# MCG-NJU/LinK

Measured on AMD Instinct MI355X. Metric: voxels/s through one LinK (3x7)^3 block, 100k active voxels C=64, higher is better.
Workload: dtype f32

## Files before the change

include/link_amd.h:

```cpp
#ifndef LINK_AMD_H_
#define LINK_AMD_H_

#include <stddef.h>
#include <stdint.h>

#ifdef __cplusplus
extern "C" {
#endif

#define LINK_OK 0
#define LINK_ERR_ARG (-1)
#define LINK_ERR_LAUNCH (-2)
#define LINK_ERR_WORKSPACE (-3)
#define LINK_BATCH_TIMEOUT (-4)

int link_abi_version(void);
int32_t link_abi_struct_size(int32_t which);
const char *link_last_error(void);


int link_hash(const int32_t *coords, int64_t n, int64_t *out, void *stream);

int link_kernel_hash(const int32_t *coords, int64_t n, const int32_t *offsets, int64_t k,
                     int64_t *out, void *stream);
// ... 427 lines not shown
  int32_t subm;
  int32_t *nbr;
  int32_t *pair_arena;
  int64_t pair_arena_words;
  float *contrib;
  int64_t contrib_rows;
  const float *w;
  const void *ws;
  const int32_t *w_big;
  const float *nl_w, *nl_b;
  float nl_eps;
  int32_t flags;
  void *out;
  int32_t bbox[8];
  int32_t stats[4];
  int32_t verdict;
  int32_t reserved;
} link_block_args_t;
int link_elk_block_forward(link_block_ctx_t *ctx, link_block_args_t *args , void *stream);

typedef struct link_dc_batch link_dc_batch_t;
int link_dc_batch_create(link_dc_batch_t **out);
int link_dc_batch_destroy(link_dc_batch_t *ctx);
int link_elk_core_dense_forward_batch(link_dc_batch_t *ctx, const link_dc_buffers_t *frames ,
                                      const int64_t *n , int32_t nframes, const link_dc_grid_t *g ,
                                      const link_elk_desc_t *desc , void *stream);
int link_dc_batch_submit(link_dc_batch_t *ctx, const link_dc_buffers_t *frames , const int64_t *n ,
                         int32_t nframes, const link_dc_grid_t *g , const link_elk_desc_t *desc , void *stream,
                         int64_t *ticket );
int link_dc_batch_join(link_dc_batch_t *ctx, int64_t ticket, void *stream);
int link_dc_batch_status(link_dc_batch_t *ctx, int32_t *out );
int link_dc_batch_set_timing(link_dc_batch_t *ctx, int32_t on);
int link_dc_batch_kernel_times(link_dc_batch_t *ctx, int64_t ticket, float *ms );
int link_dc_batch_set_debug(link_dc_batch_t *ctx, uint64_t *k1_rows, uint64_t *k2_rows);
int link_streams_share_queue(void *stream_a, void *stream_b, double *delay_us );
int link_dc_batch_probe_streams(link_dc_batch_t *ctx, hipStream_t stream, double *delays_us );

#define LINK_NMS_ROTATE 0
#define LINK_NMS_NORMAL 1
#define LINK_NMS_CIRCLE 2
int link_boxes_overlap_bev(const float *boxes_a, int64_t na, const float *boxes_b, int64_t nb, float *out , void *stream);
int link_boxes_iou_bev(const float *boxes_a, int64_t na, const float *boxes_b, int64_t nb, float *out , void *stream);
size_t link_nms_workspace_bytes(int64_t n);
int link_nms_mask(const float *boxes, int64_t cap, const int32_t *n_dev, int32_t pred, float thr, uint64_t *mask, void *stream);
int link_nms_reduce(const uint64_t *mask, int64_t cap, const int32_t *n_dev, int32_t post_max, int64_t *keep ,
                    int32_t *count , void *stream);
int link_nms_bev(const float *boxes, int64_t cap, const int32_t *n_dev, int32_t pred, float thr, int32_t post_max, void *workspace,
                 size_t workspace_bytes, int64_t *keep , int32_t *count , void *stream);
typedef struct {
  float out_size_factor, voxel_size[2], pc_range[2], score_threshold, post_center_range[6];
} link_center_geom_t;
int link_center_decode(const float *hm, const float *reg, const float *height, const float *dim, const float *rot, const float *vel,
                       int32_t batch, int32_t num_cls, int32_t h, int32_t w, const link_center_geom_t *geom , float *boxes,
                       int32_t *labels, float *scores, int32_t *counts, void *stream);

#define LINK_VOXELIZE_HARD 0
#define LINK_VOXELIZE_DYNAMIC 1
typedef struct {
  float lo[3], hi[3], vs[3];
  int32_t grid[3];
  int32_t max_points, max_voxels, ndim, mode;
} link_voxelize_geom_t;
size_t link_voxelize_workspace_bytes(const link_voxelize_geom_t *geom , int64_t n_points_capacity, int32_t batch);
int link_voxelize(const link_voxelize_geom_t *geom , const float *points, const int32_t *point_offsets ,
                  int32_t batch, int64_t n_points_capacity, void *workspace, size_t workspace_bytes, float *voxels ,
                  float *mean, int32_t *coors , int32_t *num_points, int64_t voxel_capacity,
// ... 144 lines not shown
```

link_amd/_lib.py:

```python
from __future__ import annotations

import ctypes
import os
from ctypes import POINTER, Structure, c_char_p, c_double, c_float, c_int, c_int32, c_int64, c_size_t, c_void_p

_HERE = os.path.dirname(os.path.abspath(__file__))
SO_PATH = os.path.join(_HERE, "lib", "liblink_amd.so")

LINK_OK, LINK_ERR_ARG, LINK_ERR_LAUNCH, LINK_ERR_WORKSPACE, LINK_BATCH_TIMEOUT = 0, -1, -2, -3, -4
HDR_M, HDR_STATUS, HDR_NVALID, HDR_STATUS_ACC, HDR_WORDS = 0, 1, 2, 3, 8
OP_COS, OP_SIN, OP_COSX = 0, 1, 2
ELK_LANE_CHANNEL, ELK_NO_PAIR, ELK_FUSED_GATHER, ELK_NO_DENSE_GRID, ELK_TILES = 1, 2, 4, 8, 16
ELK_LEAN_CS, ELK_LEAN_NO_CS, ELK_LEAN_PM, ELK_LEAN_NO_PM = 32, 64, 128, 256
IO_F32, IO_F16, IO_BF16 = 0, 1, 2
ABI_VERSION = 13
DEBUG = os.environ.get("LINK_AMD_DEBUG", "0") not in ("", "0")


class LinkGrid(Structure):
    _fields_ = [("s", c_int32), ("lo", c_int32 * 4), ("dim", c_int32 * 4)]

    @property
    def cells(self) -> int:
        v = 1
# ... 255 lines not shown
    "link_bn_apply_backward_io": (c_int, [c_void_p, c_void_p, c_int32] + [c_void_p] * 4 + [c_int64, c_int32, c_void_p, c_void_p]),
    "link_elk_mid_partial_rows": (c_int32, []),
    "link_dc_grid_from": (c_int64, [POINTER(LinkGrid), c_int32, POINTER(LinkDcGrid)]),
    "link_dc_premix_insert": (c_int, [c_void_p] * 5 + [c_int64, c_int32, c_float, POINTER(LinkDcGrid), c_int32] +
                              [c_void_p] * 7),
    "link_dc_modsum": (c_int, [c_void_p] * 6 + [POINTER(LinkElkDesc), POINTER(LinkDcGrid), c_int32, c_void_p,
                               c_void_p, c_void_p]),
    "link_dc_gather": (c_int, [c_void_p, c_void_p, POINTER(LinkElkDesc), POINTER(LinkDcGrid), c_void_p, c_void_p]),
    "link_elk_core_dense_forward": (c_int, [POINTER(LinkDcBuffers), POINTER(LinkDcGrid), POINTER(LinkElkDesc),
                                            c_int64, c_int32, c_void_p]),
    "link_elk_core_lean_forward": (c_int, [POINTER(LinkLeanBuffers), POINTER(LinkGrid), POINTER(LinkElkDesc), c_int64, c_int64,
                                           c_int32, c_void_p]),
    "link_dc_index_probe": (c_int, [POINTER(LinkDcBuffers), POINTER(LinkDcGrid), c_int64, c_void_p, c_void_p]),
    "link_dc_index_ids": (c_int, [c_void_p, c_int64, POINTER(LinkDcGrid)] + [c_void_p] * 5),
    "link_dc_index": (c_int, [c_void_p, c_int64, POINTER(LinkDcGrid)] + [c_void_p] * 5),
    "link_dc_premix_modsum": (c_int, [POINTER(LinkDcBuffers), POINTER(LinkDcGrid), POINTER(LinkElkDesc), c_int64,
                                      c_int32, c_void_p]),
    "link_dc_gather_demod": (c_int, [POINTER(LinkDcBuffers), POINTER(LinkDcGrid), POINTER(LinkElkDesc), c_int64, c_void_p]),
    "link_dc_demod": (c_int, [c_void_p] * 8 + [POINTER(LinkElkDesc), POINTER(LinkDcGrid), c_int64, c_void_p, c_int32,
                              c_void_p]),
    "link_block_ctx_create": (c_int, [POINTER(c_void_p)]),
    "link_block_ctx_destroy": (c_int, [c_void_p]),
    "link_pair_plan_arena": (c_int64, [c_int64, c_int32, c_int32, POINTER(c_int64)]),
    "link_dc_neighbor_map": (c_int, [c_void_p, c_int64, POINTER(LinkDcGrid), c_void_p, c_void_p, c_int32, c_void_p, c_void_p]),
    "link_elk_block_forward": (c_int, [c_void_p, POINTER(LinkBlockArgs), c_void_p]),
    "link_dc_batch_create": (c_int, [POINTER(c_void_p)]),
    "link_dc_batch_destroy": (c_int, [c_void_p]),
    "link_elk_core_dense_forward_batch": (c_int, [c_void_p, POINTER(LinkDcBuffers), POINTER(c_int64), c_int32, POINTER(LinkDcGrid),
                                                  POINTER(LinkElkDesc), c_void_p]),
    "link_dc_batch_submit": (c_int, [c_void_p, POINTER(LinkDcBuffers), POINTER(c_int64), c_int32, POINTER(LinkDcGrid),
                                     POINTER(LinkElkDesc), c_void_p, POINTER(c_int64)]),
    "link_dc_batch_join": (c_int, [c_void_p, c_int64, c_void_p]),
    "link_dc_batch_set_timing": (c_int, [c_void_p, c_int32]),
    "link_dc_batch_kernel_times": (c_int, [c_void_p, c_int64, POINTER(c_float)]),
    "link_dc_batch_status": (c_int, [c_void_p, POINTER(c_int32)]),
    "link_dc_batch_set_debug": (c_int, [c_void_p, c_void_p, c_void_p]),
    "link_dc_batch_probe_streams": (c_int, [c_void_p, c_void_p, POINTER(ctypes.c_double)]),
    "link_streams_share_queue": (c_int, [c_void_p, c_void_p, POINTER(ctypes.c_double)]),
    "link_elk_mid_backward": (c_int, [c_void_p] * 9 + [POINTER(LinkGrid), c_void_p, c_void_p, c_void_p,
                                      POINTER(LinkElkDesc), c_int64, c_int64] + [c_void_p] * 5),
    "link_boxes_overlap_bev": (c_int, [c_void_p, c_int64, c_void_p, c_int64, c_void_p, c_void_p]),
    "link_boxes_iou_bev": (c_int, [c_void_p, c_int64, c_void_p, c_int64, c_void_p, c_void_p]),
    "link_nms_workspace_bytes": (c_size_t, [c_int64]),
    "link_nms_mask": (c_int, [c_void_p, c_int64, c_void_p, c_int32, c_float, c_void_p, c_void_p]),
    "link_nms_reduce": (c_int, [c_void_p, c_int64, c_void_p, c_int32, c_void_p, c_void_p, c_void_p]),
    "link_nms_bev": (c_int, [c_void_p, c_int64, c_void_p, c_int32, c_float, c_int32, c_void_p, c_size_t, c_void_p, c_void_p, c_void_p]),
    "link_center_decode": (c_int, [c_void_p] * 6 + [c_int32] * 4 + [POINTER(LinkCenterGeom)] + [c_void_p] * 5),
    "link_voxelize_workspace_bytes": (c_size_t, [POINTER(LinkVoxelizeGeom), c_int64, c_int32]),
    "link_voxelize": (c_int, [POINTER(LinkVoxelizeGeom), c_void_p, c_void_p, c_int32, c_int64, c_void_p, c_size_t] + [c_void_p] * 4 +
                      [c_int64, c_void_p, c_void_p]),
    "link_segloss_workspace_bytes": (c_size_t, [c_int64, c_int32]),
    "link_segloss_forward": (c_int, [c_void_p, c_int32, c_int32, c_void_p, c_int64, c_int32, c_int64, c_int64, c_int32, c_int32, c_void_p,
                                     c_size_t, c_void_p, c_void_p, c_void_p]),
    "link_segloss_backward": (c_int, [c_void_p, c_void_p, c_int64, c_int32, c_int32, c_void_p, c_void_p]),
    "link_center_assign": (c_int, [POINTER(LinkCenterAssignGeom), c_void_p, c_void_p, c_int32, c_int32] + [POINTER(c_void_p)] * 5 + [c_void_p]),
    "link_center_loss_workspace_bytes": (c_size_t, [c_int32] * 5),
    "link_center_loss_forward": (c_int, [c_void_p] * 6 + [POINTER(c_int64), c_int32, c_int32] + [c_void_p] * 5 + [c_int32] * 5 + [POINTER(c_float), c_float, c_void_p,
                                         c_size_t, c_void_p, c_void_p, c_void_p, c_void_p]),
    "link_center_loss_backward": (c_int, [c_void_p] * 5 + [c_int32] * 6 + [c_void_p] * 6 + [POINTER(c_int64), c_void_p]),
    "link_seg_quantize_workspace_bytes": (c_size_t, [c_int64, c_int32]),
    "link_seg_quantize": (c_int, [c_void_p, c_int32, c_int32, c_float, c_void_p, c_int32, c_int64, c_void_p, c_size_t, c_void_p, c_void_p,
                                  c_int64] + [c_void_p] * 5),
    "link_seg_vote_eval": (c_int, [c_void_p, c_int32, c_int32, c_int64, c_int32, c_void_p, c_int32, c_int64, c_void_p, c_int64] +
                           [c_void_p] * 4),
    "link_tta_views": (c_int, [c_void_p, c_void_p, c_int32, c_int64, c_int32, c_float, c_float, c_void_p, c_void_p, c_void_p]),
    "link_center_decode_flip4": (c_int, [c_void_p] * 6 + [c_int32] * 4 + [POINTER(LinkCenterGeom)] + [c_void_p] * 5),
# ... 84 lines not shown
```

link_amd/csrc/dense_batch.hip:

```cpp
#define DC_IO 0
#define DC_IO_NS dcb_f32
#include "dense_batch_impl.h"

namespace dcb_f16 { int batch_set_launch(const link::dc_bt_host_t &, const link_dc_buffers_t *, const int64_t *, int, const link_dc_grid_t &, const link_elk_desc_t &); }
namespace dcb_bf16 { int batch_set_launch(const link::dc_bt_host_t &, const link_dc_buffers_t *, const int64_t *, int, const link_dc_grid_t &, const link_elk_desc_t &); }

using namespace link;
using namespace dcb_f32;

static constexpr int BT_RING = 4;
__global__ void k_dc_batch_spin(unsigned long long *stamp, int ticks) {
  const unsigned long long t0 = __builtin_amdgcn_s_memrealtime();
  if (threadIdx.x == 0) *stamp = t0;
  while (__builtin_amdgcn_s_memrealtime() - t0 < (unsigned long long)ticks) __builtin_amdgcn_s_sleep(16);
}
static bool bt_queue_delay_us(hipStream_t x, hipStream_t y, unsigned long long *scratch , hipEvent_t ev, double *us) {
  unsigned long long h[2] = {0, 0};
  *us = 0.0;
  if (hipStreamSynchronize(x) != hipSuccess || hipStreamSynchronize(y) != hipSuccess) return false;
  hipLaunchKernelGGL(k_dc_batch_spin, dim3(1), dim3(64), 0, x, scratch, 15000);
  if (hipEventRecord(ev, x) != hipSuccess) return false;
  hipLaunchKernelGGL(k_dc_batch_spin, dim3(1), dim3(64), 0, y, scratch + 1, 0);
  if (hipStreamSynchronize(x) != hipSuccess || hipStreamSynchronize(y) != hipSuccess ||
      hipMemcpy(h, scratch, sizeof h, hipMemcpyDeviceToHost) != hipSuccess)
    return false;
  *us = ((double)h[1] - (double)h[0]) / 100.0;
  return true;
}
static bool bt_share_queue(hipStream_t x, hipStream_t y, unsigned long long *scratch, hipEvent_t ev) {
  double d = 0.0;
  return !bt_queue_delay_us(x, y, scratch, ev, &d) || d > 75.0;
}
struct link_dc_batch {
  int device, cus;
  hipStream_t sa, sb, sc;
  std::vector<hipStream_t> pool;
  int ia, ib;
  std::vector<std::pair<hipStream_t, unsigned>> callers;
  unsigned long long *probe_scratch;
  hipEvent_t probe_ev;
  bool timing;
  hipEvent_t tb[BT_RING][3], te[BT_RING][3];
  bool timed[BT_RING];
  int32_t *sync;
  hipEvent_t ev_in[BT_RING], ev_ms[BT_RING], ev_a[BT_RING], ev_c[BT_RING], ev_out[BT_RING];
  std::vector<const void *> bufs[BT_RING];
  bool used[BT_RING];
  long long calls;
  unsigned long long *dbg1, *dbg2;
};

extern "C" int link_dc_batch_create(link_dc_batch_t **out) {
  if (!out) return LINK_ERR_ARG;
  link_dc_batch *c = new link_dc_batch();
  hipDeviceProp_t pr;
  if (hipGetDevice(&c->device) != hipSuccess || hipGetDeviceProperties(&pr, c->device) != hipSuccess) { delete c; return LINK_ERR_LAUNCH; }
  c->cus = pr.multiProcessorCount;
  int pr_lo = 0, pr_hi = 0;
  (void)hipDeviceGetStreamPriorityRange(&pr_lo, &pr_hi);
  bool ok = hipStreamCreateWithPriority(&c->sc, hipStreamNonBlocking, pr_hi) == hipSuccess &&
            hipMalloc(reinterpret_cast<void **>(&c->probe_scratch), 16) == hipSuccess &&
            hipEventCreateWithFlags(&c->probe_ev, hipEventDisableTiming) == hipSuccess;
  std::vector<hipStream_t> rejected;
  const bool dbg_place = getenv("LINK_DC_BATCH_DEBUG") != nullptr;
  for (int cand = 0; ok && cand < 12 && c->pool.size() < 4; cand++) {
    hipStream_t s_ = nullptr;
    if (hipStreamCreateWithFlags(&s_, hipStreamNonBlocking) != hipSuccess) { ok = false; break; }
    bool bad = bt_share_queue(c->sc, s_, c->probe_scratch, c->probe_ev);
    for (size_t i = 0; i < c->pool.size() && !bad; i++) bad = bt_share_queue(c->pool[i], s_, c->probe_scratch, c->probe_ev);
    (bad ? rejected : c->pool).push_back(s_);
  }
  while (ok && c->pool.size() < 2 && !rejected.empty()) { c->pool.push_back(rejected.back()); rejected.pop_back(); }
  for (hipStream_t s_ : rejected) (void)hipStreamDestroy(s_);
  ok = ok && c->pool.size() >= 2;
  if (ok) { c->ia = 0; c->ib = 1; c->sa = c->pool[0]; c->sb = c->pool[1]; }
  if (dbg_place)
    fprintf(stderr, "link_dc_batch_create: %zu streams on hardware queues of their own, %zu candidates rejected\n",
            c->pool.size(), rejected.size());
  ok = ok && hipMalloc(reinterpret_cast<void **>(&c->sync), sizeof(int32_t) * BT_RING * BT_SYNC_WORDS) == hipSuccess &&
            hipMemset(c->sync, 0, sizeof(int32_t) * BT_RING * BT_SYNC_WORDS) == hipSuccess;
  for (int i = 0; i < BT_RING && ok; i++) {
#ifndef DC_BT_EVENT_FLAGS
#define DC_BT_EVENT_FLAGS (hipEventDisableTiming | hipEventDisableSystemFence)
#endif
    ok = hipEventCreateWithFlags(&c->ev_in[i], DC_BT_EVENT_FLAGS) == hipSuccess && hipEventCreateWithFlags(&c->ev_ms[i], DC_BT_EVENT_FLAGS) == hipSuccess &&
         hipEventCreateWithFlags(&c->ev_a[i], DC_BT_EVENT_FLAGS) == hipSuccess && hipEventCreateWithFlags(&c->ev_c[i], DC_BT_EVENT_FLAGS) == hipSuccess &&
         hipEventCreateWithFlags(&c->ev_out[i], DC_BT_EVENT_FLAGS) == hipSuccess;
    c->used[i] = false;
  }
  c->calls = 0;
  c->dbg1 = c->dbg2 = nullptr;
  if (!ok) { (void)hipGetLastError(); delete c; return LINK_ERR_LAUNCH; }
  *out = c;
  return LINK_OK;
}

extern "C" int link_dc_batch_destroy(link_dc_batch_t *c) {
  if (!c) return LINK_OK;
  (void)hipStreamSynchronize(c->sa); (void)hipStreamSynchronize(c->sb); (void)hipStreamSynchronize(c->sc);
  for (int i = 0; i < BT_RING; i++) {
    (void)hipEventDestroy(c->ev_in[i]); (void)hipEventDestroy(c->ev_ms[i]); (void)hipEventDestroy(c->ev_a[i]); (void)hipEventDestroy(c->ev_c[i]);
    (void)hipEventDestroy(c->ev_out[i]);
  }
  for (int i = 0; i < BT_RING; i++)
    for (int k = 0; k < 3; k++) { if (c->tb[i][k]) (void)hipEventDestroy(c->tb[i][k]); if (c->te[i][k]) (void)hipEventDestroy(c->te[i][k]); }
  (void)hipFree(c->sync);
  (void)hipFree(c->probe_scratch);
  (void)hipEventDestroy(c->probe_ev);
  for (hipStream_t s_ : c->pool) (void)hipStreamDestroy(s_);
  (void)hipStreamDestroy(c->sc);
  delete c;
  return LINK_OK;
}

extern "C" int link_dc_batch_set_debug(link_dc_batch_t *c, uint64_t *k1_rows, uint64_t *k2_rows) {
  if (!c) return LINK_ERR_ARG;
  c->dbg1 = reinterpret_cast<unsigned long long *>(k1_rows);
  c->dbg2 = reinterpret_cast<unsigned long long *>(k2_rows);
  return DC_BT_PROF ? LINK_OK : 1;
}

extern "C" int link_streams_share_queue(void *a, void *b, double *delay_us) {
  if (!delay_us) return LINK_ERR_ARG;
  unsigned long long *st = nullptr;
  hipEvent_t ev;
  if (hipMalloc(reinterpret_cast<void **>(&st), 16) != hipSuccess) return LINK_ERR_LAUNCH;
  if (hipEventCreateWithFlags(&ev, hipEventDisableTiming) != hipSuccess) { (void)hipFree(st); return LINK_ERR_LAUNCH; }
  const bool ok = bt_queue_delay_us(S(a), S(b), st, ev, delay_us);
  (void)hipEventDestroy(ev);
  (void)hipFree(st);
  if (!ok) { (void)hipGetLastError(); return LINK_ERR_LAUNCH; }
  return LINK_OK;
}

extern "C" int link_dc_batch_probe_streams(link_dc_batch_t *c, hipStream_t caller, double *delays_us ) {
  if (!c || !delays_us) return LINK_ERR_ARG;
  unsigned long long *st = nullptr;
  hipEvent_t ev;
  if (hipMalloc(reinterpret_cast<void **>(&st), 16) != hipSuccess) return LINK_ERR_LAUNCH;
  if (hipEventCreateWithFlags(&ev, hipEventDisableTiming) != hipSuccess) { (void)hipFree(st); return LINK_ERR_LAUNCH; }
  hipStream_t xs[12] = {c->sa, c->sa, c->sb, caller, caller, caller, c->sb, c->sc, c->sc, c->sa, c->sb, c->sc},
              ys[12] = {c->sb, c->sc, c->sc, c->sa, c->sb, c->sc, c->sa, c->sa, c->sb, caller, caller, caller};
  bool ok = true;
  for (int i = 0; i < 12; i++) ok = bt_queue_delay_us(xs[i], ys[i], st, ev, &delays_us[i]) && ok;
// ... 93 lines not shown
    for (int i = 0; i < nb; i++) keys.push_back(frames[base + i].S);
    bool fail = hipEventRecord(c->ev_in[q], st) != hipSuccess;
    fail = fail || hipStreamWaitEvent(c->sa, c->ev_in[q], 0) != hipSuccess || hipStreamWaitEvent(c->sb, c->ev_in[q], 0) != hipSuccess ||
           hipStreamWaitEvent(c->sc, c->ev_in[q], 0) != hipSuccess;
    for (int r = 0; r < BT_RING && !fail; r++) {
      if (!c->used[r]) continue;
      bool dep = r == q;
      for (size_t i = 0; i < keys.size() && !dep; i++)
        for (size_t k = 0; k < c->bufs[r].size() && !dep; k++) dep = keys[i] == c->bufs[r][k];
      if (dep)
        fail = hipStreamWaitEvent(c->sa, c->ev_out[r], 0) != hipSuccess || hipStreamWaitEvent(c->sc, c->ev_out[r], 0) != hipSuccess ||
               hipStreamWaitEvent(c->sa, c->ev_a[r], 0) != hipSuccess || hipStreamWaitEvent(c->sc, c->ev_a[r], 0) != hipSuccess;
    }
    int32_t *sync = c->sync + (size_t)q * BT_SYNC_WORDS;
#ifndef DC_BT_CLEAR_ON_INSERT
#define DC_BT_CLEAR_ON_INSERT 1
#endif
    hipStream_t s_clear = DC_BT_CLEAR_ON_INSERT ? c->sc : c->sa, s_o1 = DC_BT_CLEAR_ON_INSERT ? c->sa : c->sc;
    if (!fail) hipLaunchKernelGGL(k_dc_batch_clear, dim3(1), dim3(256), 0, s_clear, sync, (int)BT_SYNC_WORDS);
    fail = fail || hipEventRecord(c->ev_ms[q], s_clear) != hipSuccess ||
           hipStreamWaitEvent(c->sb, c->ev_ms[q], 0) != hipSuccess || hipStreamWaitEvent(s_o1, c->ev_ms[q], 0) != hipSuccess;
    if (fail) { (void)hipGetLastError(); return LINK_ERR_LAUNCH; }
    int rc;
    hipStream_t role3[3] = {c->sc, c->sa, c->sb};
    c->timed[q] = false;
    if (c->timing) {
      bool okt = true;
      for (int i = 0; i < 3 && okt; i++) {
        if (!c->tb[q][i]) okt = hipEventCreate(&c->tb[q][i]) == hipSuccess && hipEventCreate(&c->te[q][i]) == hipSuccess;
        okt = okt && hipEventRecord(c->tb[q][i], role3[i]) == hipSuccess;
      }
      c->timed[q] = okt;
    }
    const dc_bt_host_t hset{c->sa, c->sb, c->sc, c->cus, sync, c->dbg1, c->dbg2};
    if (b0.io_dtype == LINK_IO_F16) rc = dcb_f16::batch_set_launch(hset, frames + base, n + base, nb, *g, *d);
    else if (b0.io_dtype == LINK_IO_BF16) rc = dcb_bf16::batch_set_launch(hset, frames + base, n + base, nb, *g, *d);
    else rc = dcb_f32::batch_set_launch(hset, frames + base, n + base, nb, *g, *d);
    if (c->timed[q])
      for (int i = 0; i < 3; i++) c->timed[q] = hipEventRecord(c->te[q][i], role3[i]) == hipSuccess && c->timed[q];
    fail = hipEventRecord(c->ev_a[q], c->sa) != hipSuccess || hipEventRecord(c->ev_c[q], c->sc) != hipSuccess || hipEventRecord(c->ev_out[q], c->sb) != hipSuccess;
    c->bufs[q] = keys;
    c->used[q] = true;
    if (ticket) *ticket = c->calls;
    c->calls++;
    if (rc != LINK_OK || fail) {
      (void)hipStreamWaitEvent(st, c->ev_a[q], 0); (void)hipStreamWaitEvent(st, c->ev_c[q], 0); (void)hipStreamWaitEvent(st, c->ev_out[q], 0);
      if (rc != LINK_OK) return rc;
      (void)hipGetLastError();
      return LINK_ERR_LAUNCH;
    }
  }
  return LINK_OK;
}

extern "C" int link_dc_batch_join(link_dc_batch_t *c, int64_t ticket, void *stream) {
  if (!c || ticket < 0 || ticket >= c->calls) return LINK_ERR_ARG;
  const int q = (int)(ticket % BT_RING);
  hipStream_t st = S(stream);
  if (hipStreamWaitEvent(st, c->ev_a[q], 0) != hipSuccess || hipStreamWaitEvent(st, c->ev_c[q], 0) != hipSuccess ||
      hipStreamWaitEvent(st, c->ev_out[q], 0) != hipSuccess) {
    (void)hipGetLastError();
    return LINK_ERR_LAUNCH;
  }
  return LINK_OK;
}

extern "C" int link_elk_core_dense_forward_batch(link_dc_batch_t *c, const link_dc_buffers_t *frames, const int64_t *n, int32_t nframes,
// ... 7 lines not shown
```

link_amd/csrc/dense_batch_common.h:

```cpp
#pragma once
#include <hip/hip_runtime.h>
#include <stdint.h>

#include "link_amd.h"

#ifndef DC_BT_MAX
#define DC_BT_MAX 48
#endif
#ifndef DC_BT_TIMEOUT_TICKS
#define DC_BT_TIMEOUT_TICKS 200000000ull
#endif
#ifndef DC_BT_PROF
#define DC_BT_PROF 0
#endif
#ifndef DC_BT_INS_LEAD
#define DC_BT_INS_LEAD 1000
#endif
#ifndef DC_BT_INS_WAVES
#define DC_BT_INS_WAVES 4
#endif
#ifndef DC_BT_RELEASE_FENCE
#define DC_BT_RELEASE_FENCE 0
#endif
#ifndef DC_BT_K1_WRITEBACK
#define DC_BT_K1_WRITEBACK 0
#endif

namespace link {
__host__ __device__ constexpr int bt_err() { return 0; }
__host__ __device__ constexpr int bt_cursor(int xcd) { return 16 * (1 + xcd); }
__host__ __device__ constexpr int bt_k1cur(int xcd) { return 16 * (9 + xcd); }
__host__ __device__ constexpr int bt_inscur() { return 16 * 17; }
__host__ __device__ constexpr int bt_ins(int f) { return 16 * (18 + 2 * f); }
__host__ __device__ constexpr int bt_k1(int f) { return 16 * (19 + 2 * f); }
constexpr int BT_SYNC_WORDS = 16 * (18 + 2 * DC_BT_MAX);
struct dc_bt_host_t {
  hipStream_t sa, sb, sc;
  int cus;
  int32_t *sync;
  unsigned long long *dbg1, *dbg2;
};
}
```

link_amd/csrc/dense_batch_impl.h:

```cpp
#include <stdlib.h>

#include <type_traits>
#include <vector>

#include "dense_batch_common.h"
#include "dense_gather.h"
#include "dense_io.h"

namespace DC_IO_NS {
using namespace link;

#include "dense_k1_impl.h"
#include "dense_k2_cfg.h"
#include "dense_gather_quad_impl.h"

static_assert(DC_ST_AUX == 16, "the S rows must leave the L2 (sc1) for the in-launch hand-off K1 -> K2");

struct dc_bt_frame_t {
  const void *feats; const int4 *coords; int4 *slots; uint32_t *cnt; int32_t *cell_n; int32_t *vcell; float *S; int32_t *hdr;
  void *out; int64_t n;
};
struct dc_bt_frames_t { dc_bt_frame_t f[DC_BT_MAX]; };
struct dc_bt_par_t {
  const float *w_pre, *pre_ln_w, *pre_ln_b, *w_pos, *ln_w, *ln_b;
  int cg; float eps;
  unsigned long long *dbg1, *dbg2;
};
__device__ __forceinline__ void bt_row(unsigned long long *dbg, unsigned long long r, unsigned long long a, unsigned long long b,
                                       unsigned long long c, unsigned long long d, unsigned long long e, unsigned long long f) {
  if (!DC_BT_PROF || !dbg) return;
  if (r + 1 >= dbg[1]) return;
  unsigned long long *o = dbg + 8 * (r + 1);
  o[0] = a; o[1] = b; o[2] = c; o[3] = d; o[4] = e; o[5] = f; o[6] = 1;
}


template <typename P>
__device__ __forceinline__ bool bt_wait_ge(P sync, int word, int target, const int nap = 8) {
  int ok = 1;
  if ((threadIdx.x & 63) == 0) {
    const unsigned long long t0 = __builtin_amdgcn_s_memrealtime();
    int spins = 0;
    while (__hip_atomic_load(&sync[word], __ATOMIC_RELAXED, __HIP_MEMORY_SCOPE_AGENT) < target) {
      if (nap > 8) __builtin_amdgcn_s_sleep(64); else __builtin_amdgcn_s_sleep(8);
      if ((++spins & 15) == 0) {
        if (__hip_atomic_load(&sync[bt_err()], __ATOMIC_RELAXED, __HIP_MEMORY_SCOPE_AGENT) != 0) { ok = 0; break; }
        if (__builtin_amdgcn_s_memrealtime() - t0 > DC_BT_TIMEOUT_TICKS) {
          __hip_atomic_store(&sync[bt_err()], 1 + word, __ATOMIC_RELAXED, __HIP_MEMORY_SCOPE_AGENT);
          ok = 0;
          break;
        }
      }
    }
  }
  return __builtin_amdgcn_readfirstlane(ok) != 0;
}

struct dc_bt_ins_args_t { dc_bt_frames_t fr; link_dc_grid_t g; int nframes, wpf; int32_t *sync; };
__global__ void __launch_bounds__(64) k_dc_batch_insert(dc_bt_ins_args_t args_by_value) {
  (void)args_by_value;
#if defined(__HIP_DEVICE_COMPILE__)
  typedef const __attribute__((address_space(4))) dc_bt_ins_args_t *args_ptr_t;
  for (;;) {
    args_ptr_t a = (args_ptr_t)__builtin_amdgcn_kernarg_segment_ptr();
    asm volatile("" : "+s"(a));
    int t = 0;
    if (threadIdx.x == 0) t = __hip_atomic_fetch_add(&a->sync[bt_inscur()], 1, __ATOMIC_RELAXED, __HIP_MEMORY_SCOPE_AGENT);
    t = __builtin_amdgcn_readfirstlane(t);
    const int wpf = a->wpf;
    if (t >= a->nframes * wpf) break;
    const int f = t / wpf, j = t - f * wpf;
    if (f >= DC_BT_INS_LEAD && !bt_wait_ge(a->sync, bt_k1(f - DC_BT_INS_LEAD), 1, 64)) break;
    const link_dc_grid_t g = a->g;
    const int n = (int)a->fr.f[f].n;
    const int4 *__restrict__ coords = a->fr.f[f].coords;
    int32_t *__restrict__ vcell = a->fr.f[f].vcell;
    int32_t *__restrict__ hdr = a->fr.f[f].hdr;
    const __amdgpu_buffer_rsrc_t r_slots = dc_rsrc(a->fr.f[f].slots, (uint32_t)((int64_t)g.vp * g.k * 16));
    const __amdgpu_buffer_rsrc_t r_cnt = dc_rsrc(a->fr.f[f].cnt, (uint32_t)(g.vp * 4));
    if (j == 0 && threadIdx.x == 0) hdr[LINK_HDR_NVALID] = n;
    _Pragma("unroll 1") for (int k = 0; k < 4; k++) {
      const int v = (4 * j + k) * 64 + (int)threadIdx.x;
      if (v >= n) break;
      const int4 rc = coords[v];
      const unsigned ux = (unsigned)(floordiv(rc.x, g.s) - g.lo[0]), uy = (unsigned)(floordiv(rc.y, g.s) - g.lo[1]);
      const unsigned uz = (unsigned)(floordiv(rc.z, g.s) - g.lo[2]), ub = (unsigned)(rc.w - g.lo[3]);
      const bool inside = ux < (unsigned)g.dim[0] && uy < (unsigned)g.dim[1] && uz < (unsigned)g.dim[2] && ub < (unsigned)g.dim[3];
      if (!inside) atomicOr(&hdr[LINK_HDR_STATUS_ACC], 1);
      const int pcell = inside ? dc_cell(g, (int)ux, (int)uy, (int)uz, (int)ub) : 0;
      const int rank = __builtin_amdgcn_raw_ptr_buffer_atomic_add_i32(1, r_cnt, pcell ? (uint32_t)pcell * 4u : DC_OOB, 0, 0);
      const bool full = pcell != 0 && rank >= g.k;
      if (full) atomicOr(&hdr[LINK_HDR_STATUS_ACC], 2);
      const bool keep = pcell != 0 && !full;
      st16i_c<true>(r_slots, keep ? dc_slot(g, pcell, rank) * 16u : DC_OOB, make_int4(rc.x, rc.y, rc.z, v));
      vcell[v] = keep ? pcell : 0;
    }
    asm volatile("s_waitcnt vmcnt(0)" ::: "memory");
    if (threadIdx.x == 0) __hip_atomic_fetch_add(&a->sync[bt_ins(f)], 1, __ATOMIC_RELAXED, __HIP_MEMORY_SCOPE_AGENT);
  }
#endif
}

template <int OP, int NB>
__global__ void __launch_bounds__(64 * DC_K1_NW, DC_K1_WAVES) k_dc_batch_k1(dc_bt_frames_t fr, dc_bt_par_t p, link_dc_grid_t g, int nframes,
                                                                           int cpw, int nranges, int wpf, int32_t *__restrict__ sync) {
  constexpr int C = 64;
  extern __shared__ __attribute__((aligned(16))) char smem_raw[];
  const int tid = threadIdx.x, lane = tid & 63;
  bool w_big = false, th_big = false;
  dc_k1_stage<C, OP>(smem_raw, p.w_pre, p.pre_ln_w, p.pre_ln_b, p.w_pos, nullptr, p.cg, 1.0f, g, tid, w_big, th_big);
  w_big = DC_K1_SPLIT ? (__syncthreads_or(w_big) != 0) : (__syncthreads(), false);
  const bool th_slow = DC_THETA_BOUND ? __syncthreads_or(th_big) != 0 : false;
  const int Vi = g.dim[0] * g.dim[1] * g.dim[2] * g.dim[3];
  const int x = (int)(__builtin_amdgcn_s_getreg((4 - 1) << 11 | 0 << 6 | 20) & 7u);
  const int per = (nranges + 7) >> 3;
  const int lo = x * per;
  const int mine = (lo + per < nranges ? lo + per : nranges) - lo;
  if (mine <= 0) return;
  const int total = nframes * mine;
  int32_t *cur = &sync[bt_k1cur(x)];
  int t_next = 0;
  if (lane == 0) t_next = __hip_atomic_fetch_add(cur, 1, __ATOMIC_RELAXED, __HIP_MEMORY_SCOPE_AGENT);
  int pend_f = -1;
  int ins_known = -1;
  for (;;) {
    const int t = __builtin_amdgcn_readfirstlane(t_next);
    if (t >= total) break;
    const unsigned long long tp0 = DC_BT_PROF ? __builtin_amdgcn_s_memrealtime() : 0;
    const int f = t / mine, i = lo + (t - f * mine);
    if (lane == 0) t_next = __hip_atomic_fetch_add(cur, 1, __ATOMIC_RELAXED, __HIP_MEMORY_SCOPE_AGENT);
    const dc_bt_frame_t &F = fr.f[f];
    int ins_a = wpf, ins_b = wpf;
    if (lane == 0) {
      if (f > ins_known) ins_a = __hip_atomic_load(&sync[bt_ins(f)], __ATOMIC_RELAXED, __HIP_MEMORY_SCOPE_AGENT);
      if (f + 1 < nframes && f + 1 > ins_known) ins_b = __hip_atomic_load(&sync[bt_ins(f + 1)], __ATOMIC_RELAXED, __HIP_MEMORY_SCOPE_AGENT);
    }
    const int c_begin = i * cpw;
    const int c_end = (c_begin + cpw < Vi) ? c_begin + cpw : Vi;
    int pc_f, nv_f;
    int4 rf0, rf1, rf2, rf3;
    if (f <= ins_known) dc_k1_prefetch<true>(pc_f, nv_f, rf0, rf1, rf2, rf3, g, F.slots, F.cnt, c_begin, c_end, lane);
    asm volatile("s_waitcnt vmcnt(0)" ::: "memory");
    if (pend_f >= 0 && lane == 0) __hip_atomic_fetch_add(&sync[bt_k1(pend_f)], 1, __ATOMIC_RELAXED, __HIP_MEMORY_SCOPE_AGENT);
    pend_f = f;
    if (f > ins_known) {
      if (__builtin_amdgcn_readfirstlane(ins_a) < wpf && !bt_wait_ge(sync, bt_ins(f), wpf)) return;
      ins_known = f;
      dc_k1_prefetch<true>(pc_f, nv_f, rf0, rf1, rf2, rf3, g, F.slots, F.cnt, c_begin, c_end, lane);
    }
    if (f + 1 < nframes && f + 1 > ins_known && __builtin_amdgcn_readfirstlane(ins_b) >= wpf) ins_known = f + 1;
    if (i == 0 && lane == 0) {
      F.hdr[LINK_HDR_STATUS] = __hip_atomic_load(&F.hdr[LINK_HDR_STATUS_ACC], __ATOMIC_RELAXED, __HIP_MEMORY_SCOPE_AGENT);
      __hip_atomic_store(&F.hdr[LINK_HDR_STATUS_ACC], 0, __ATOMIC_RELAXED, __HIP_MEMORY_SCOPE_AGENT);
    }
    const unsigned long long tp1 = DC_BT_PROF ? __builtin_amdgcn_s_memrealtime() : 0;
    dc_k1_range<C, OP, NB, false, true, DC_BT_K1_WRITEBACK != 0>(smem_raw, F.feats, F.slots, F.cnt, F.cell_n, p.w_pre, 1.0f, p.eps, F.n, g, false, F.S, nullptr,
                                        nullptr, c_begin, c_end, pc_f, nv_f, rf0, rf1, rf2, rf3, w_big, th_slow, i, 0, 0);
    if (DC_BT_PROF && lane == 0) bt_row(p.dbg1, (unsigned long long)f * nranges + i, (unsigned long long)f, (unsigned long long)i, tp0, tp1, __builtin_amdgcn_s_memrealtime(), (unsigned long long)(blockIdx.x * 4 + (tid >> 6)));
  }
  asm volatile("s_waitcnt vmcnt(0)" ::: "memory");
#if DC_BT_RELEASE_FENCE
  __builtin_amdgcn_fence(__ATOMIC_RELEASE, "agent");
  asm volatile("s_waitcnt vmcnt(0)" ::: "memory");
#endif
  if (pend_f >= 0 && lane == 0) __hip_atomic_fetch_add(&sync[bt_k1(pend_f)], 1, __ATOMIC_RELAXED, __HIP_MEMORY_SCOPE_AGENT);
}

struct dc_bt_k2_args_t {
  dc_bt_frames_t fr;
  dc_bt_par_t p;
  link_dc_grid_t g;
  int nframes, txn, tyn, zsplit, nwg, k1_target;
  int32_t *sync;
};

template <int OP, int R>
__global__ void __launch_bounds__(256 + 64 * (DC_K2Q_CW + (DC_K2Q_PMAP ? 1 : 0)), 4) k_dc_batch_k2(dc_bt_k2_args_t args_by_value) {
  (void)args_by_value;
#if defined(__HIP_DEVICE_COMPILE__)
  static_assert(DC_K2Q_PMAP == 1, "the mapper wave draws the items");
  typedef const __attribute__((address_space(4))) dc_bt_k2_args_t *args_ptr_t;
  constexpr unsigned CTL_THREAD = 256 + 64 * DC_K2Q_CW;
  __shared__ int s_ctl[4];
// ... 42 lines not shown
    __syncthreads();
  }
#endif
}


template <int OP, int R>
static int batch_launch(const dc_bt_host_t &c, const dc_bt_frames_t &fr, const dc_bt_par_t &p, const link_dc_grid_t &g, const link_elk_desc_t &d,
                        int nframes, int64_t nmax, bool strips) {
  using K1 = dc_k1_cfg<64, OP>;
  using KQ = dc_k2q_cfg<OP, R>;
  constexpr int LDS_GRAN = 1280, LDS_GRANS = 128, K1_STATIC = 256, K2_STATIC = 16;
  constexpr int k1_lds = 65 * LDS_GRAN - K1_STATIC;
  constexpr int k2_lds = KQ::LDS_BYTES;
  static_assert(k1_lds >= K1::LDS_BYTES && (k2_lds + K2_STATIC + LDS_GRAN - 1) / LDS_GRAN <= LDS_GRANS - 65, "LDS shaping of the two persistent roles");
  int32_t *sync = c.sync;
  const int64_t vi = (int64_t)g.dim[0] * g.dim[1] * g.dim[2] * g.dim[3];
  const int k1_wgs = c.cus;
  static const int rpw = [] { const char *e = getenv("LINK_DC_BATCH_RPW"); const int v = e ? atoi(e) : 1; return v < 1 ? 1 : (v > 16 ? 16 : v); }();
  int cpw = (int)((vi + (int64_t)k1_wgs * K1::NW * rpw - 1) / ((int64_t)k1_wgs * K1::NW * rpw));
  if (cpw < 1) cpw = 1;
  const int k1_target = (int)((vi + cpw - 1) / cpw);
  const dc_k2q_tiles_t tq = dc_k2q_tiles(g, R, strips);
  static const int zs_env = [] { const char *e = getenv("LINK_DC_BATCH_ZSPLIT"); const int v = e ? atoi(e) : 1; return v < 1 ? 1 : (v > 8 ? 8 : v); }();
  int zsplit = zs_env;
  if (zsplit > g.dim[2]) zsplit = g.dim[2];
  const int64_t nwg = ((int64_t)tq.txn * tq.tyn + tq.nxs + tq.nys) * g.dim[3] * zsplit;
  if (nwg > (1 << 20)) return LINK_ERR_ARG;
  int wpf = (int)((nmax + 255) / 256);
  if (wpf < 1) wpf = 1;
  (void)hipFuncSetAttribute(reinterpret_cast<const void *>(&k_dc_batch_k1<OP, 2>), hipFuncAttributeMaxDynamicSharedMemorySize, k1_lds);
  (void)hipFuncSetAttribute(reinterpret_cast<const void *>(&k_dc_batch_k2<OP, R>), hipFuncAttributeMaxDynamicSharedMemorySize, k2_lds);
  const int ins_wgs = c.cus;
  const dc_bt_ins_args_t a0{fr, g, nframes, wpf, sync};
  hipLaunchKernelGGL(k_dc_batch_insert, dim3((unsigned)ins_wgs * DC_BT_INS_WAVES), dim3(64), 0, c.sc, a0);
  int rc = check_launch("link_elk_core_dense_forward_batch (insert)");
  if (rc != LINK_OK) return rc;
  hipLaunchKernelGGL((k_dc_batch_k1<OP, 2>), dim3((unsigned)k1_wgs), dim3(64 * K1::NW), k1_lds, c.sa, fr, p, g, nframes, cpw, k1_target, wpf, sync);
  rc = check_launch("link_elk_core_dense_forward_batch (K1)");
  if (rc != LINK_OK) return rc;
  const dc_bt_k2_args_t a2{fr, p, g, nframes, tq.txn, tq.tyn, zsplit, (int)nwg, k1_target, sync};
  static_assert(sizeof(dc_bt_k2_args_t) <= 4096, "kernel arguments");
  hipLaunchKernelGGL((k_dc_batch_k2<OP, R>), dim3((unsigned)c.cus), dim3(KQ::THREADS), k2_lds, c.sb, a2);
  return check_launch("link_elk_core_dense_forward_batch (K2)");
}

int batch_set_launch(const dc_bt_host_t &c, const link_dc_buffers_t *frames, const int64_t *n, int nb, const link_dc_grid_t &g,
                     const link_elk_desc_t &d) {
  const link_dc_buffers_t &b0 = frames[0];
  const dc_bt_par_t p{b0.w_pre, b0.pre_ln_w, b0.pre_ln_b, b0.w_pos, b0.ln_w, b0.ln_b, d.cg, d.eps, c.dbg1, c.dbg2};
  dc_bt_frames_t fr{};
  int64_t nmax = 0;
  for (int i = 0; i < nb; i++) {
    const link_dc_buffers_t &b = frames[i];
    fr.f[i] = dc_bt_frame_t{b.feats, reinterpret_cast<const int4 *>(b.coords), reinterpret_cast<int4 *>(b.slots), b.cnt, b.cell_n, b.vcell, b.S,
                            b.hdr, b.out, n[i]};
    nmax = n[i] > nmax ? n[i] : nmax;
  }
  static const bool sq_env = [] { const char *e = getenv("LINK_DC_BATCH_SQUARE_RIM"); return e && atoi(e) != 0; }();
  const bool strips = !(b0.tune.k2_form & 16) && !sq_env;
  if (d.op == LINK_OP_COS) return d.r == 3 ? batch_launch<LINK_OP_COS, 3>(c, fr, p, g, d, nb, nmax, strips) : batch_launch<LINK_OP_COS, 2>(c, fr, p, g, d, nb, nmax, strips);
  return d.r == 3 ? batch_launch<LINK_OP_SIN, 3>(c, fr, p, g, d, nb, nmax, strips) : batch_launch<LINK_OP_SIN, 2>(c, fr, p, g, d, nb, nmax, strips);
}
}
```

link_amd/elk.py:

```python
from __future__ import annotations

import ctypes
import weakref
import math
from typing import Dict, Optional, Tuple

import torch
import torch.nn as nn
import torch.nn.functional as TF

from . import _lib as L
from .aggregate import _AuxToVoxel, _BlockMean, link_index_of
from .functional import sphash, sphashquery
from .index import BlockIndex, GridTooLarge, box_neighbor_map, foreign_neighbor_map, strided_out_coords, transpose_table
from .tensor import SparseTensor
from .utils import get_kernel_offsets, make_ntuple

__all__ = ["ELKBlock", "TSELKBlock", "Conv3d", "spconv2ts", "ts2spconv", "SparseConvTensor",
           "elk_core_fused", "elk_core_autograd", "elk_core_train", "ElkCorePlan", "subm_conv", "subm_conv_ln_add_relu",
           "invalidate_derived_weights", "release_block_driver"]

_OPS = {"cos": L.OP_COS, "sin": L.OP_SIN, "cos_x": L.OP_COSX}
_IO_DTYPES = {torch.float32: L.IO_F32, torch.float16: L.IO_F16, torch.bfloat16: L.IO_BF16}

# ... 532 lines not shown
        if L.DEBUG:
            self.check()
        return res

    def submit(self, feats, coords, outs=None, stream: Optional[int] = None):
        k, res = self._fill(feats, coords, outs)
        p0 = self.plans[0]
        st = L.current_stream_handle() if stream is None else int(stream)
        ticket = ctypes.c_int64(-1)
        rc = L.lib().link_dc_batch_submit(self._ctx, self._bufs, self._n, k, ctypes.byref(p0.dcg), ctypes.byref(p0.desc), st, ctypes.byref(ticket))
        if rc != 0:
            L.check(rc, "link_dc_batch_submit")
        return res, int(ticket.value)

    def join(self, ticket: int, stream: Optional[int] = None) -> None:
        st = L.current_stream_handle() if stream is None else int(stream)
        rc = L.lib().link_dc_batch_join(self._ctx, int(ticket), st)
        if rc != 0:
            L.check(rc, "link_dc_batch_join")
        if L.DEBUG:
            self.check()

    def check(self) -> None:
        st = (ctypes.c_int32 * 2)()
        rc = L.lib().link_dc_batch_status(self._ctx, st)
        if rc != 0:
            raise L.LinkAmdError(f"ElkCoreBatch: link_dc_batch_status = {rc} (error word {st[0]}: a persistent kernel's bounded "
                                 "wait gave up; the batch's rows are undefined)")
        for p in self.plans:
            p.check()

    def set_timing(self, on: bool) -> None:
        L.check(L.lib().link_dc_batch_set_timing(self._ctx, 1 if on else 0), "link_dc_batch_set_timing")

    def kernel_times_us(self, ticket: int):
        out = (ctypes.c_float * 3)()
        L.check(L.lib().link_dc_batch_kernel_times(self._ctx, int(ticket), out), "link_dc_batch_kernel_times")
        return [1e3 * float(v) for v in out]

    def probe_streams(self, stream: Optional[int] = None):
        out = (ctypes.c_double * 12)()
        L.check(L.lib().link_dc_batch_probe_streams(self._ctx, stream if stream is not None else _st(), out), "link_dc_batch_probe_streams")
        return [round(float(v), 1) for v in out]

    def arena_bytes(self) -> int:
        return sum(p.arena_bytes() for p in self.plans)


def _aggregate(x: torch.Tensor, index: BlockIndex, r: int) -> torch.Tensor:
    mean = _BlockMean.apply(x, index)
    return _AuxToVoxel.apply(mean, index.counts, None, index.idx_query, index, r)


def elk_core_autograd(feats, coords, index, w_pre, pre_ln_w, pre_ln_b, w_pos, alpha, ln_w, ln_b, baseop,
                      cg, r, coord_div=1.0, eps=1e-6):
    c = feats.shape[1]
    fin = TF.layer_norm(TF.linear(feats, w_pre), (c,), pre_ln_w, pre_ln_b, eps)
    xyz = coords[:, :3].float()
    if coord_div != 1.0:
        xyz = xyz / coord_div
    th = TF.linear(xyz, w_pos)
    if alpha is not None:
        th = th * alpha
    if c != cg:
        th = th.repeat([1, c // cg])
    sin, cos = torch.sin(th), torch.cos(th)
# ... 1571 lines not shown
```

Baseline: 3.330 billion.

## Pace batch insert kernel by K1 demand signal instead of fixed lead wait

```diff
diff --git a/include/link_amd.h b/include/link_amd.h
--- a/include/link_amd.h
+++ b/include/link_amd.h
@@ -483,6 +483,7 @@
 int link_dc_batch_status(link_dc_batch_t *ctx, int32_t *out );
 int link_dc_batch_set_timing(link_dc_batch_t *ctx, int32_t on);
 int link_dc_batch_kernel_times(link_dc_batch_t *ctx, int64_t ticket, float *ms );
+int link_dc_batch_set_insert_pacing(link_dc_batch_t *ctx, int32_t active_waves, int32_t nap_us, int32_t lead);
 int link_dc_batch_set_debug(link_dc_batch_t *ctx, uint64_t *k1_rows, uint64_t *k2_rows);
 int link_streams_share_queue(void *stream_a, void *stream_b, double *delay_us );
 int link_dc_batch_probe_streams(link_dc_batch_t *ctx, hipStream_t stream, double *delays_us );
diff --git a/link_amd/_lib.py b/link_amd/_lib.py
--- a/link_amd/_lib.py
+++ b/link_amd/_lib.py
@@ -311,6 +311,7 @@
                                      POINTER(LinkElkDesc), c_void_p, POINTER(c_int64)]),
     "link_dc_batch_join": (c_int, [c_void_p, c_int64, c_void_p]),
     "link_dc_batch_set_timing": (c_int, [c_void_p, c_int32]),
+    "link_dc_batch_set_insert_pacing": (c_int, [c_void_p, c_int32, c_int32, c_int32]),
     "link_dc_batch_kernel_times": (c_int, [c_void_p, c_int64, POINTER(c_float)]),
     "link_dc_batch_status": (c_int, [c_void_p, POINTER(c_int32)]),
     "link_dc_batch_set_debug": (c_int, [c_void_p, c_void_p, c_void_p]),
diff --git a/link_amd/csrc/dense_batch.hip b/link_amd/csrc/dense_batch.hip
--- a/link_amd/csrc/dense_batch.hip
+++ b/link_amd/csrc/dense_batch.hip
@@ -48,6 +48,8 @@
   bool used[BT_RING];
   long long calls;
   unsigned long long *dbg1, *dbg2;
+  int ins_act, ins_nap, ins_lead;
+  int ins_act0, ins_nap0, ins_lead0;
 };
 
 extern "C" int link_dc_batch_create(link_dc_batch_t **out) {
@@ -90,6 +92,12 @@
   }
   c->calls = 0;
   c->dbg1 = c->dbg2 = nullptr;
+  c->ins_act = DC_BT_INS_ACT < 0 ? c->cus : DC_BT_INS_ACT; c->ins_nap = DC_BT_INS_NAP; c->ins_lead = DC_BT_INS_LEADF;
+  if (const char *e = getenv("LINK_DC_BATCH_INS_PACING")) {
+    int v[3] = {c->ins_act, c->ins_nap, c->ins_lead};
+    if (sscanf(e, "%d,%d,%d", &v[0], &v[1], &v[2]) >= 1 && v[0] >= 0) (void)link_dc_batch_set_insert_pacing(c, v[0], v[1], v[2]);
+  }
+  c->ins_act0 = c->ins_act; c->ins_nap0 = c->ins_nap; c->ins_lead0 = c->ins_lead;
   if (!ok) { (void)hipGetLastError(); delete c; return LINK_ERR_LAUNCH; }
   *out = c;
   return LINK_OK;
@@ -110,6 +118,15 @@
   for (hipStream_t s_ : c->pool) (void)hipStreamDestroy(s_);
   (void)hipStreamDestroy(c->sc);
   delete c;
+  return LINK_OK;
+}
+
+extern "C" int link_dc_batch_set_insert_pacing(link_dc_batch_t *c, int32_t active_waves, int32_t nap_us, int32_t lead) {
+  if (!c) return LINK_ERR_ARG;
+  if (active_waves < 0) { c->ins_act = c->ins_act0; c->ins_nap = c->ins_nap0; c->ins_lead = c->ins_lead0; return LINK_OK; }
+  c->ins_act = active_waves;
+  c->ins_nap = nap_us < 0 ? 0 : (nap_us > DC_BT_INS_NAP_MAX ? DC_BT_INS_NAP_MAX : nap_us);
+  c->ins_lead = lead < 0 ? 0 : (lead > DC_BT_MAX ? DC_BT_MAX : lead);
   return LINK_OK;
 }
 
@@ -269,7 +286,7 @@
       }
       c->timed[q] = okt;
     }
-    const dc_bt_host_t hset{c->sa, c->sb, c->sc, c->cus, sync, c->dbg1, c->dbg2};
+    const dc_bt_host_t hset{c->sa, c->sb, c->sc, c->cus, sync, c->dbg1, c->dbg2, c->ins_act, c->ins_nap, c->ins_lead};
     if (b0.io_dtype == LINK_IO_F16) rc = dcb_f16::batch_set_launch(hset, frames + base, n + base, nb, *g, *d);
     else if (b0.io_dtype == LINK_IO_BF16) rc = dcb_bf16::batch_set_launch(hset, frames + base, n + base, nb, *g, *d);
     else rc = dcb_f32::batch_set_launch(hset, frames + base, n + base, nb, *g, *d);
diff --git a/link_amd/csrc/dense_batch_common.h b/link_amd/csrc/dense_batch_common.h
--- a/link_amd/csrc/dense_batch_common.h
+++ b/link_amd/csrc/dense_batch_common.h
@@ -13,9 +13,16 @@
 #ifndef DC_BT_PROF
 #define DC_BT_PROF 0
 #endif
-#ifndef DC_BT_INS_LEAD
-#define DC_BT_INS_LEAD 1000
+#ifndef DC_BT_INS_ACT
+#define DC_BT_INS_ACT (-1)
 #endif
+#ifndef DC_BT_INS_NAP
+#define DC_BT_INS_NAP 0
+#endif
+#ifndef DC_BT_INS_LEADF
+#define DC_BT_INS_LEADF 4
+#endif
+#define DC_BT_INS_NAP_MAX 10000
 #ifndef DC_BT_INS_WAVES
 #define DC_BT_INS_WAVES 4
 #endif
@@ -33,11 +40,13 @@
 __host__ __device__ constexpr int bt_inscur() { return 16 * 17; }
 __host__ __device__ constexpr int bt_ins(int f) { return 16 * (18 + 2 * f); }
 __host__ __device__ constexpr int bt_k1(int f) { return 16 * (19 + 2 * f); }
-constexpr int BT_SYNC_WORDS = 16 * (18 + 2 * DC_BT_MAX);
+__host__ __device__ constexpr int bt_need() { return 16 * (18 + 2 * DC_BT_MAX); }
+constexpr int BT_SYNC_WORDS = 16 * (19 + 2 * DC_BT_MAX);
 struct dc_bt_host_t {
   hipStream_t sa, sb, sc;
   int cus;
   int32_t *sync;
   unsigned long long *dbg1, *dbg2;
+  int ins_act, ins_nap, ins_lead;
 };
 }
diff --git a/link_amd/csrc/dense_batch_impl.h b/link_amd/csrc/dense_batch_impl.h
--- a/link_amd/csrc/dense_batch_impl.h
+++ b/link_amd/csrc/dense_batch_impl.h
@@ -56,21 +56,88 @@
   return __builtin_amdgcn_readfirstlane(ok) != 0;
 }
 
-struct dc_bt_ins_args_t { dc_bt_frames_t fr; link_dc_grid_t g; int nframes, wpf; int32_t *sync; };
+struct dc_bt_ins_args_t { dc_bt_frames_t fr; link_dc_grid_t g; int nframes, wpf; int32_t *sync; int act, nap, lead, k1_rows; unsigned long long *dbg; };
+constexpr int BT_NEED_DONE = 1 << 20;
+constexpr unsigned long long BT_NEED_REREAD_TICKS = 2500;
 __global__ void __launch_bounds__(64) k_dc_batch_insert(dc_bt_ins_args_t args_by_value) {
   (void)args_by_value;
 #if defined(__HIP_DEVICE_COMPILE__)
   typedef const __attribute__((address_space(4))) dc_bt_ins_args_t *args_ptr_t;
+  int full_to = -1;
+  int last_f = -1;
+  unsigned t_need = 0;
+  bool need_read = false;
+  const unsigned long long tk0 = DC_BT_PROF ? __builtin_amdgcn_s_memrealtime() : 0;
+  unsigned long long tk1 = 0;
+  int n_items = 0;
   for (;;) {
     args_ptr_t a = (args_ptr_t)__builtin_amdgcn_kernarg_segment_ptr();
     asm volatile("" : "+s"(a));
+    const int wpf = a->wpf;
+    const bool paced = a->act > 0 || a->nap > 0;
+    const bool drawer = a->act <= 0 || (int)blockIdx.x < a->act;
+    if (paced && !drawer && last_f >= full_to) {
+      int go = 1;
+      if (threadIdx.x == 0) {
+        const unsigned long long t0 = __builtin_amdgcn_s_memrealtime();
+        for (;;) {
+          const int need = __hip_atomic_load(&a->sync[bt_need()], __ATOMIC_RELAXED, __HIP_MEMORY_SCOPE_AGENT);
+          if (need >= BT_NEED_DONE) { go = 0; break; }
+          if (need > 0 && need - 1 + a->lead > last_f) { full_to = need - 1 + a->lead; break; }
+          if (__hip_atomic_load(&a->sync[bt_err()], __ATOMIC_RELAXED, __HIP_MEMORY_SCOPE_AGENT) != 0) { go = 0; break; }
+          if (__builtin_amdgcn_s_memrealtime() - t0 > DC_BT_TIMEOUT_TICKS) {
+            __hip_atomic_store(&a->sync[bt_err()], 1 + bt_need(), __ATOMIC_RELAXED, __HIP_MEMORY_SCOPE_AGENT);
+            go = 0;
+            break;
+          }
+          _Pragma("unroll 1") for (int k = 0; k < 32; k++) __builtin_amdgcn_s_sleep(127);
+        }
+      }
+      full_to = __builtin_amdgcn_readfirstlane(full_to);
+      if (__builtin_amdgcn_readfirstlane(go) == 0) break;
+    }
     int t = 0;
     if (threadIdx.x == 0) t = __hip_atomic_fetch_add(&a->sync[bt_inscur()], 1, __ATOMIC_RELAXED, __HIP_MEMORY_SCOPE_AGENT);
     t = __builtin_amdgcn_readfirstlane(t);
-    const int wpf = a->wpf;
-    if (t >= a->nframes * wpf) break;
+    if (t >= a->nframes * wpf) {
+      if (paced && threadIdx.x == 0) (void)__hip_atomic_fetch_max(&a->sync[bt_need()], BT_NEED_DONE, __ATOMIC_RELAXED, __HIP_MEMORY_SCOPE_AGENT);
+      break;
+    }
     const int f = t / wpf, j = t - f * wpf;
-    if (f >= DC_BT_INS_LEAD && !bt_wait_ge(a->sync, bt_k1(f - DC_BT_INS_LEAD), 1, 64)) break;
+    last_f = f;
+    bool thin = false;
+    if (paced && drawer && f > full_to && a->nap == 0 && need_read && (unsigned)__builtin_amdgcn_s_memrealtime() - t_need < (unsigned)BT_NEED_REREAD_TICKS) {
+      thin = true;
+    } else if (paced && drawer && f > full_to) {
+      int go = 1;
+      if (threadIdx.x == 0) {
+        const unsigned long long t0 = __builtin_amdgcn_s_memrealtime(), nap_ticks = 100ull * (unsigned long long)a->nap;
+        unsigned long long t_read = t0;
+        for (;;) {
+          const int need = __hip_atomic_load(&a->sync[bt_need()], __ATOMIC_RELAXED, __HIP_MEMORY_SCOPE_AGENT);
+          if (need > 0) full_to = need - 1 + a->lead;
+          if (f <= full_to) break;
+          unsigned long long now = __builtin_amdgcn_s_memrealtime();
+          if (now - t0 >= nap_ticks) { go = 2; break; }
+          if (__hip_atomic_load(&a->sync[bt_err()], __ATOMIC_RELAXED, __HIP_MEMORY_SCOPE_AGENT) != 0) { go = 0; break; }
+          if (now - t0 > DC_BT_TIMEOUT_TICKS) {
+            __hip_atomic_store(&a->sync[bt_err()], 1 + bt_need(), __ATOMIC_RELAXED, __HIP_MEMORY_SCOPE_AGENT);
+            go = 0;
+            break;
+          }
+          const unsigned long long t_next = t_read + BT_NEED_REREAD_TICKS < t0 + nap_ticks ? t_read + BT_NEED_REREAD_TICKS : t0 + nap_ticks;
+          while ((now = __builtin_amdgcn_s_memrealtime()) < t_next) { if (t_next - now > 340) __builtin_amdgcn_s_sleep(127); else __builtin_amdgcn_s_sleep(8); }
+          t_read = now;
+        }
+      }
+      full_to = __builtin_amdgcn_readfirstlane(full_to);
+      go = __builtin_amdgcn_readfirstlane(go);
+      t_need = (unsigned)__builtin_amdgcn_s_memrealtime();
+      need_read = true;
+      if (go == 0) break;
+      thin = go == 2;
+    }
+    if (DC_BT_PROF) { tk1 = __builtin_amdgcn_s_memrealtime(); n_items += thin ? 0x10001 : 1; }
     const link_dc_grid_t g = a->g;
     const int n = (int)a->fr.f[f].n;
     const int4 *__restrict__ coords = a->fr.f[f].coords;
@@ -97,6 +164,11 @@
     }
     asm volatile("s_waitcnt vmcnt(0)" ::: "memory");
     if (threadIdx.x == 0) __hip_atomic_fetch_add(&a->sync[bt_ins(f)], 1, __ATOMIC_RELAXED, __HIP_MEMORY_SCOPE_AGENT);
+  }
+  if (DC_BT_PROF && threadIdx.x == 0) {
+    args_ptr_t a = (args_ptr_t)__builtin_amdgcn_kernarg_segment_ptr();
+    if (n_items > 0)
+      bt_row(a->dbg, (unsigned long long)a->nframes * a->k1_rows + blockIdx.x, 9998, (unsigned long long)(n_items & 0xFFFF), tk0, tk1, __builtin_amdgcn_s_memrealtime(), (unsigned long long)(n_items >> 16));
   }
 #endif
 }
@@ -144,11 +216,23 @@
     if (pend_f >= 0 && lane == 0) __hip_atomic_fetch_add(&sync[bt_k1(pend_f)], 1, __ATOMIC_RELAXED, __HIP_MEMORY_SCOPE_AGENT);
     pend_f = f;
     if (f > ins_known) {
-      if (__builtin_amdgcn_readfirstlane(ins_a) < wpf && !bt_wait_ge(sync, bt_ins(f), wpf)) return;
+      if (__builtin_amdgcn_readfirstlane(ins_a) < wpf) {
+        if (lane == 0) {
+          (void)__hip_atomic_fetch_max(&sync[bt_need()], f + 1, __ATOMIC_RELAXED, __HIP_MEMORY_SCOPE_AGENT);
+          if (DC_BT_PROF && p.dbg1) atomicAdd(&p.dbg1[2], 1ull);
+        }
+        if (!bt_wait_ge(sync, bt_ins(f), wpf)) return;
+      }
       ins_known = f;
       dc_k1_prefetch<true>(pc_f, nv_f, rf0, rf1, rf2, rf3, g, F.slots, F.cnt, c_begin, c_end, lane);
     }
-    if (f + 1 < nframes && f + 1 > ins_known && __builtin_amdgcn_readfirstlane(ins_b) >= wpf) ins_known = f + 1;
+    if (f + 1 < nframes && f + 1 > ins_known) {
+      if (__builtin_amdgcn_readfirstlane(ins_b) >= wpf) ins_known = f + 1;
+      else if (lane == 0) {
+        (void)__hip_atomic_fetch_max(&sync[bt_need()], f + 2, __ATOMIC_RELAXED, __HIP_MEMORY_SCOPE_AGENT);
+        if (DC_BT_PROF && p.dbg1) atomicAdd(&p.dbg1[2], 1ull);
+      }
+    }
     if (i == 0 && lane == 0) {
       F.hdr[LINK_HDR_STATUS] = __hip_atomic_load(&F.hdr[LINK_HDR_STATUS_ACC], __ATOMIC_RELAXED, __HIP_MEMORY_SCOPE_AGENT);
       __hip_atomic_store(&F.hdr[LINK_HDR_STATUS_ACC], 0, __ATOMIC_RELAXED, __HIP_MEMORY_SCOPE_AGENT);
@@ -257,7 +341,8 @@
   (void)hipFuncSetAttribute(reinterpret_cast<const void *>(&k_dc_batch_k1<OP, 2>), hipFuncAttributeMaxDynamicSharedMemorySize, k1_lds);
   (void)hipFuncSetAttribute(reinterpret_cast<const void *>(&k_dc_batch_k2<OP, R>), hipFuncAttributeMaxDynamicSharedMemorySize, k2_lds);
   const int ins_wgs = c.cus;
-  const dc_bt_ins_args_t a0{fr, g, nframes, wpf, sync};
+  const dc_bt_ins_args_t a0{fr, g, nframes, wpf, sync, c.ins_act, c.ins_nap, c.ins_lead, k1_target, c.dbg1};
+  static_assert(sizeof(dc_bt_ins_args_t) <= 4096, "kernel arguments");
   hipLaunchKernelGGL(k_dc_batch_insert, dim3((unsigned)ins_wgs * DC_BT_INS_WAVES), dim3(64), 0, c.sc, a0);
   int rc = check_launch("link_elk_core_dense_forward_batch (insert)");
   if (rc != LINK_OK) return rc;
diff --git a/link_amd/elk.py b/link_amd/elk.py
--- a/link_amd/elk.py
+++ b/link_amd/elk.py
@@ -588,6 +588,9 @@
 
     def set_timing(self, on: bool) -> None:
         L.check(L.lib().link_dc_batch_set_timing(self._ctx, 1 if on else 0), "link_dc_batch_set_timing")
+
+    def set_insert_pacing(self, active_waves: int, nap_us: int, lead: int) -> None:
+        L.check(L.lib().link_dc_batch_set_insert_pacing(self._ctx, int(active_waves), int(nap_us), int(lead)), "link_dc_batch_set_insert_pacing")
 
     def kernel_times_us(self, ticket: int):
         out = (ctypes.c_float * 3)()
```

Result: no change. 3.318 billion (-0.4%).
